# ml-inory/whisper.axera

Hardware: AMD Instinct MI355X
Metric: clips_per_sec (30 s clips, greedy decode, whisper-small) (higher is better)
Workload: dtype bf16; 1 GPU; whisper-small bf16, batch 1/GPU, 30 s synthetic 16 kHz clips resident in HBM, greedy decode 444 ids/clip (448 decoder steps); batch_per_gpu=1, global_batch=1, parallelism=dp1, weights=seeded synthetic, collective=none

## Files before the change

### whisper.axera_amd/csrc/common.hpp

```cpp
#pragma once

#include <hip/hip_runtime.h>
#include <stdint.h>

#ifndef AXW_F16
#define AXW_F16 0
#endif
#if AXW_F16
#define AXW_NS hf
#else
#define AXW_NS bf
#endif

namespace axw {
inline namespace AXW_NS {

#if AXW_F16
typedef _Float16 h16;
constexpr const char* kDtypeName = "fp16";
#else
typedef __bf16 h16;
constexpr const char* kDtypeName = "bf16";
#endif
typedef h16 h16x4 __attribute__((ext_vector_type(4)));
// ... 289 lines not shown
  float* amax_val; int* amax_idx; int amax_stride;
  float* logits_dump; long logits_dump_stride;
  int skip_before_step;
  int ksplit; int part_batch;
};
void launch_decode_gemm(const DecGemmParams& p, hipStream_t s);

struct DecCGemmParams {
  const h16* W;
  const float* bias; int N, K, batch;
  const float* x; const float* ln_w; const float* ln_b;
  const h16* a_hi; const h16* a_lo;
  int nbs;
  int epilogue;
  int rt;
  float* out;
  h16* out_hi; h16* out_lo;
  h16* k_cache; h16* v_cache; long kv_batch_stride; int d_model; int n_ctx_pad;
  const DecState* state;
  const int* off;
  int fold_row0;
  const float* ln_w2;
  const h16* W_lo;
  float* out2;
  float* stat_part;
  unsigned long long* stamp; int stamp_point;
};
void launch_decode_cgemm(const DecCGemmParams& p, hipStream_t s);
int decode_gemm_grid(int N, int rt);
bool decode_logits_resident_ok(int K, int batch);
void launch_act_prep(float* x, const float* g, const float* be, h16* hi, h16* lo, int batch, int K, bool do_ln, int nbs,
                     const float* part, int n_part, int part_batch, const float* part_bias, hipStream_t s);
void launch_pack_weight_frag(const h16* w, h16* wp, int N, int K, hipStream_t s);
void launch_pack_weight_frag_split(const float* w, h16* hi, h16* lo, int N, int K, hipStream_t s);

struct AdvanceParams {
  const float* amax_val; const int* amax_idx; int n_part; int amax_stride;
  DecState* state; int* off; int* tok; int* done; int* n_out; int* out_ids; int batch;
  int* done_host;
  int n_ctx, eot, max_new, n_vocab;
  const int* max_new_clip;
  const int* sot;
  const int* forced; int n_forced;
  int* argmax_dump;
  const h16* tok_emb; const float* pos; float* x; int d_model;
  int n_prefix;
};
void launch_advance(const AdvanceParams& p, hipStream_t s);

struct TsRulesParams {
  const float* logits; long stride;
  int batch, n_vocab, eot, ts_begin;
  const int* off;
  int n_prefix;
  const int* done;
  const int* out_ids; const int* n_out; int n_ctx;
  const int* forced; int n_forced;
  float* amax_val; int* amax_idx; int amax_stride;
};
void launch_timestamp_rules(const TsRulesParams& p, hipStream_t s);

typedef unsigned long long u64;
struct PersistParams {
  const h16* wl; const float* fl;
  const float* qf;
  const h16* tok_emb; const float* pos; const float* ln_w; const float* ln_b;
  const h16* cross_k; const h16* cross_v; long cross_layer_stride;
  int n_layer, n_vocab, n_ctx, n_audio_ctx;
  int eot, max_new, total_steps;
  const int* sot;
  const int* forced; int n_forced; float* logits_dump; int* argmax_dump;
  u64* gran; unsigned* err;
  int gran_bytes;
  int* out_ids; int* n_out; DecState* state;
  int fault;
  long long* prof;
  int n_clip;
  int prof_clip;
  long cross_clip_stride;
  h16* self_k1; h16* self_v1;
  long gran_clip_u64;
  int* out_ids1; int* n_out1; int max_new1;
  int max_new2; long self_clip_stride;
};
bool decode_persistent_supported(int d_model, int n_head, int n_layer, int n_cu);
int decode_persistent_grid(int d_model, int n_cu);
size_t decode_persistent_gran_bytes(int d_model, int grid);
size_t qfold_floats(int d_model, int n_layer);
void launch_qfold_build(const h16* wl, const float* fl, float* qf, int d_model, int n_layer, hipStream_t s);
hipError_t launch_decode_persistent(const PersistParams& p, int d_model, int grid, hipStream_t s);
int decode_persistent_max_clips(int d_model, int n_head, int n_layer, int grid);

void launch_convert_to_h16(const void* src, int src_dtype , h16* dst, long n, hipStream_t s);
void launch_convert_to_f32(const void* src, int src_dtype, float* dst, long n, hipStream_t s);
void launch_conv_weight_pack(const void* src, int src_dtype, h16* dst, int cout, int cin, int kpad, hipStream_t s);

}
}
```

### whisper.axera_amd/csrc/decode_persistent.hip

```cpp
#include "decode_persistent_common.hpp"

namespace axw {
inline namespace AXW_NS {

__global__ void qfold_vec_kernel(const h16* __restrict__ wl, const float* __restrict__ fl, float* __restrict__ qf, int D) {
  const int l = blockIdx.y;
  const long DD = (long)D * D;
  const h16* WL = wl + (long)l * DecArena::w_stride(D);
  const float* F = fl + (long)l * DecArena::f_stride(D);
  float* out = qf + (long)l * qfold_stride(D) + DD;
  const int j = blockIdx.x * blockDim.x + threadIdx.x;
  if (j < 3 * D) {
    const h16* w = WL + DecArena::W_QKV * DD + (long)j * D;
    const float *g = F + DecArena::F_ATTN_LN_W * D, *be = F + DecArena::F_ATTN_LN_B * D;
    double ss = 0.0, cc = 0.0;
    for (int i = 0; i < D; ++i) { const double wv = (double)(float)w[i]; ss += wv * (double)g[i]; cc += wv * (double)be[i]; }
    out[QF_SQKV * D + j] = (float)ss;
    out[QF_CQKV * D + j] = (float)(cc + (double)F[DecArena::F_B_QKV * D + j]);
  }
  if (j < 4 * D) {
    const h16* w = WL + DecArena::W_FC1 * DD + (long)j * D;
    const float *g = F + DecArena::F_MLP_LN_W * D, *be = F + DecArena::F_MLP_LN_B * D;
    double ss = 0.0, cc = 0.0;
    for (int i = 0; i < D; ++i) { const double wv = (double)(float)w[i]; ss += wv * (double)g[i]; cc += wv * (double)be[i]; }
    out[QF_SFC1 * D + j] = (float)ss;
    out[QF_CFC1 * D + j] = (float)(cc + (double)F[DecArena::F_B_FC1 * D + j]);
  }
}


__global__ void qfold_build_kernel(const h16* __restrict__ wl, const float* __restrict__ fl, float* __restrict__ qf, int D) {
  const int l = blockIdx.z;
  const long DD = (long)D * D;
  const h16* wq = wl + (long)l * DecArena::w_stride(D) + DecArena::W_CQ * DD;
  const h16* wo = wl + (long)l * DecArena::w_stride(D) + DecArena::W_O * DD;
  const float* F = fl + (long)l * DecArena::f_stride(D);
  const float *g = F + DecArena::F_CROSS_LN_W * D, *be = F + DecArena::F_CROSS_LN_B * D, *bo = F + DecArena::F_B_O * D, *bq = F + DecArena::F_B_CQ * D;
  float* out = qf + (long)l * qfold_stride(D);
  const int k = blockIdx.x * blockDim.x + threadIdx.x, j = blockIdx.y;
  if (k >= D) return;
  double acc = 0.0;
  for (int i = 0; i < D; ++i) acc += (double)(float)wq[(long)j * D + i] * (double)g[i] * (double)(float)wo[(long)i * D + k];
  out[(long)j * D + k] = (float)acc;
  if (k == 0) {
    double dd = 0.0, ss = 0.0, cc = 0.0;
    for (int i = 0; i < D; ++i) {
      const double w = (double)(float)wq[(long)j * D + i];
      dd += w * (double)g[i] * (double)bo[i];
      ss += w * (double)g[i];
      cc += w * (double)be[i];
    }
    out[DD + j] = (float)dd;
    out[DD + D + j] = (float)ss;
    out[DD + 2 * D + j] = (float)(cc + (double)bq[j]);
  }
}
void launch_qfold_build(const h16* wl, const float* fl, float* qf, int d_model, int n_layer, hipStream_t s) {
  qfold_build_kernel<<<dim3((d_model + 127) / 128, d_model, n_layer), 128, 0, s>>>(wl, fl, qf, d_model);
  qfold_vec_kernel<<<dim3((4 * d_model + 127) / 128, n_layer), 128, 0, s>>>(wl, fl, qf, d_model);
}
size_t qfold_floats(int d_model, int n_layer) { return (size_t)n_layer * (size_t)qfold_stride(d_model); }

template <int LD, int CD, int LF, int CF, bool PROF, bool QF>
__global__ __launch_bounds__(PT) void decode_persistent_kernel(PersistParams p) {
  AXW_PERSIST_SHAPES
  constexpr int XG = D, X0R = 2 * D, A0S = 3 * D;
  AXW_PERSIST_LDS(4)
  AXW_PERSIST_IDS
  const __amdgpu_buffer_rsrc_t GR = __builtin_amdgcn_make_buffer_rsrc((void*)p.gran, 0, p.gran_bytes, 0x27000);
  AXW_PERSIST_ROLES
  AXW_PERSIST_INIT
#define AXW_TL(IDX) \
  if (PROF && tl_on && (tid == 0 || tid == PL)) prof_acc[32 + (IDX)] = wall_clock64();
  int tok = AXW_COLD(sot)[0];
  int n_out = 0, n_done = 0, steps_run = 0;

  if (poller) {
    float x[GD];
    float lg[GD], lb[GD];
    float shift = 0.f;
    AXW_POLLER_PREFETCH
#define AXW_PAIRS_D(BASE) [&](int j) { const int pr = tid + j * PL; return 2 * pr < D ? (BASE) + 2 * pr : -1; }

#define AXW_RAW_STAGE(FAIL, CODE, XGW)                                                      \
  {                                                                                          \
    float s1 = 0.f, s2 = 0.f;                                                                \
    _Pragma("unroll") for (int k = 0; k < GD; ++k) {                                         \
      const int i = el(k);                                                                   \
      if (i < D) {                                                                           \
        const float t = x[k] - shift;                                                        \
        s1 += t; s2 += t * t;                                                                \
        act[i] = x[k] * lg[k];                                                               \
        if (XGW) { act[XG + i] = x[k] * g2[k]; act[X0R + i] = x[k]; }                        \
      }                                                                                      \
    }                                                                                        \
    s1 = wsum(s1); s2 = wsum(s2);                                                            \
    if ((tid & 63) == 0) { red[2 * (tid >> 6)] = s1; red[2 * (tid >> 6) + 1] = s2; }         \
    if (tid == 0) red[2 * NPW + 1] = shift;                                                  \
    if (FAIL) ctl[0] = 1;                                                                    \
    AXW_BARRIER_CHECK(CODE)                                                                  \
    float t1 = 0.f;                                                                          \
    _Pragma("unroll") for (int w2 = 0; w2 < NPW; ++w2) t1 += red[2 * w2];                    \
    shift += t1 / D;                                                                         \
    if (tid == 0) red[2 * NPW] = shift;                                                      \
  }
#define AXW_LN_STAGE(Y, ADD, FAIL, CODE) AXW_LN_STAGE_X(Y, ADD, FAIL, CODE, false)
#define AXW_LN_STAGE_X(Y, ADD, FAIL, CODE, XGW)                                             \
  {                                                                                          \
    float s1 = 0.f, s2 = 0.f;                                                                \
    _Pragma("unroll") for (int k = 0; k < GD; ++k) {                                         \
      if (el(k) < D) {                                                                       \
        if (ADD) x[k] += __uint_as_float(Y[k]);                                              \
        const float t = x[k] - shift;                                                        \
        s1 += t; s2 += t * t;                                                                \
      }                                                                                      \
    }                                                                                        \
    s1 = wsum(s1); s2 = wsum(s2);                                                            \
    if ((tid & 63) == 0) { red[2 * (tid >> 6)] = s1; red[2 * (tid >> 6) + 1] = s2; }         \
    if (FAIL) ctl[0] = 1;                                                                    \
    AXW_BARRIER_CHECK(CODE)                                                                  \
    float t1 = 0.f, t2 = 0.f;                                                                \
    _Pragma("unroll") for (int w2 = 0; w2 < NPW; ++w2) { t1 += red[2 * w2]; t2 += red[2 * w2 + 1]; } \
    const float dm = t1 / D, var = fmaxf(t2 / D - dm * dm, 0.f);                             \
    const float mean = shift + dm, rstd = rsqrtf(var + 1e-5f);                               \
    if (QF && tid == 0) red[2 * NPW] = mean;                                                 \
    _Pragma("unroll") for (int k = 0; k < GD; ++k) {                                         \
      const int i = el(k);                                                                   \
      if (i < D) act[i] = (x[k] - mean) * rstd * lg[k] + lb[k];                              \
      if (QF && (XGW) && i < D) { act[XG + i] = x[k] * g2[k]; act[X0R + i] = x[k]; }         \
    }                                                                                        \
    shift = mean;                                                                            \
    wg_barrier();                                                                            \
  }

    for (int step = 0; step < p.total_steps; ++step) {
      AXW_EMBED(x, tok)
      ln_prefetch(p.fl + DecArena::F_ATTN_LN_W * D, p.fl + DecArena::F_ATTN_LN_B * D);

      for (int l = 0; l < L; ++l) {
        asm volatile("" : "+v"(tid));
        const bool tl_on = step == p.total_steps / 2 && l == L / 2;
        const float* FL = p.fl + (long)l * DecArena::f_stride(D);
        const unsigned tag = (unsigned)(step * L + l + 1);
        {
          unsigned y[GD];
          bool fail = false;
          if (l > 0) fail = gather2<GPD>(GR, tag - 1, y, p.err, ctl, AXW_PAIRS_D(O_Y3));
          AXW_STAMP(0)
          AXW_TL(0)
          if constexpr (QF) {
            if (l > 0) {
#pragma unroll
              for (int k = 0; k < GD; ++k) if (el(k) < D) x[k] += __uint_as_float(y[k]);
            }
            AXW_RAW_STAGE(fail, 0x100 + l, in_o)
            ln_prefetch(FL + DecArena::F_MLP_LN_W * D, FL + DecArena::F_MLP_LN_B * D);
          } else {
            AXW_LN_STAGE_X(y, l > 0, fail, 0x100 + l, in_o)
            ln_prefetch(FL + DecArena::F_CROSS_LN_W * D, FL + DecArena::F_CROSS_LN_B * D);
          }
          AXW_STAMP(1)
          AXW_TL(1)
        }
        if (l == sa_layer) {
// ... 58 lines not shown
              qs[32 + tid] = lo;
            }
            if (fail) ctl[0] = 1;
          }
          AXW_STAMP(7)
          AXW_BARRIER_CHECK(0x500 + l)
          AXW_STAMP(8)
        }
        if (in_o) {
          unsigned y[2 * GP1];
          const bool fail = gather2<GP1>(GR, tag, y, p.err, ctl, [&](int j) { const int pi = tid + j * PL; return pi < NPP1 ? O_PART + (pi / (kPS / 2)) * kRec + 2 * (pi % (kPS / 2)) : -1; });
          float* pbuf = act + D;
#pragma unroll
          for (int j = 0; j < GP1; ++j) {
            const int pi = tid + j * PL;
            if (pi < NPP1) { pbuf[2 * pi] = __uint_as_float(y[2 * j]); pbuf[2 * pi + 1] = __uint_as_float(y[2 * j + 1]); }
          }
          if (fail) ctl[0] = 1;
          AXW_STAMP(9)
          AXW_TL(5)
          AXW_BARRIER_CHECK(0x600 + l)
#pragma unroll
          for (int k = 0; k < GD; ++k) {
            const int i = tid + k * PL;
            if (i < D) {
              act[i] = merge_cross_records(pbuf, i);
            }
          }
          wg_barrier();
          AXW_STAMP(10)
          AXW_TL(6)
        }
        if constexpr (QF) {
          unsigned y[2 * GD];
          const bool fail = gather2<2 * GPD>(GR, tag, y, p.err, ctl, [&](int j) { const int pr = tid + (j % GPD) * PL; return 2 * pr < D ? (j < GPD ? O_Y1 : O_Y2) + 2 * pr : -1; });
#pragma unroll
          for (int k = 0; k < GD; ++k) if (el(k) < D) x[k] = (x[k] + __uint_as_float(y[k])) + __uint_as_float(y[GD + k]);
          AXW_STAMP(11)
          AXW_TL(7)
          AXW_RAW_STAGE(fail, 0x700 + l, false)
          if (l + 1 < L) ln_prefetch(FL + DecArena::f_stride(D) + DecArena::F_ATTN_LN_W * D, FL + DecArena::f_stride(D) + DecArena::F_ATTN_LN_B * D);
          else ln_prefetch(AXW_COLD(ln_w), AXW_COLD(ln_b));
          g2_prefetch(l + 1 < L ? l + 1 : 0);
          AXW_STAMP(12)
          AXW_TL(8)
        } else {
          unsigned y[GD];
          const bool fail = gather2<GPD>(GR, tag, y, p.err, ctl, AXW_PAIRS_D(O_Y2));
          AXW_STAMP(11)
          AXW_TL(7)
          AXW_LN_STAGE(y, true, fail, 0x700 + l)
          if (l + 1 < L) ln_prefetch(FL + DecArena::f_stride(D) + DecArena::F_ATTN_LN_W * D, FL + DecArena::f_stride(D) + DecArena::F_ATTN_LN_B * D);
          else ln_prefetch(AXW_COLD(ln_w), AXW_COLD(ln_b));
          AXW_STAMP(12)
          AXW_TL(8)
        }
        if (in_f2) {
          constexpr int GH = (F / 4 + PL - 1) / PL;
          unsigned y[2 * GH];
          const bool fail = gather2<GH>(GR, tag, y, p.err, ctl, [&](int j) { const int pi = tid + j * PL; return pi < F / 4 ? O_HID + 2 * pi : -1; });
#pragma unroll
          for (int j = 0; j < GH; ++j) {
            const int pi = tid + j * PL;
            if (pi < F / 4) { act[2 * pi] = __uint_as_float(y[2 * j]); act[2 * pi + 1] = __uint_as_float(y[2 * j + 1]); }
          }
          if (fail) ctl[0] = 1;
          AXW_STAMP(13)
          AXW_TL(9)
          AXW_BARRIER_CHECK(0x800 + l)
        }
      }

      steps_run = step + 1;
      asm volatile("" : "+v"(tid));
      if (step < 3) {
        tok = AXW_COLD(sot)[step + 1];
        if constexpr (QF) wg_barrier();
        continue;
      }
      {
        unsigned y[GD];
        const bool fail = gather2<GPD>(GR, (unsigned)(step * L + L), y, p.err, ctl, AXW_PAIRS_D(O_Y3));
        AXW_LN_STAGE(y, true, fail, 0x900)
        AXW_STAMP(14)
        wg_barrier();
        unsigned v[2];
        const bool fail2 = gather2<1>(GR, (unsigned)(step + 1), v, p.err, ctl, [&](int) { return tid < P ? O_AMAX + 2 * tid : -1; });
        float cv = tid < P ? __uint_as_float(v[0]) : -INFINITY;
        int ci = tid < P ? (int)v[1] : 0x7fffffff;
        wave_argmax(cv, ci);
        if ((tid & 63) == 0) { am_v[tid >> 6] = cv; am_i[tid >> 6] = ci; }
        if (fail2) ctl[0] = 1;
        AXW_STAMP(15)
        AXW_BARRIER_CHECK(0xA00)
      }
      float cv = am_v[0];
      int best_idx = am_i[0];
      for (int w2 = 1; w2 < NPW; ++w2)
        if (am_v[w2] > cv || (am_v[w2] == cv && am_i[w2] < best_idx)) { cv = am_v[w2]; best_idx = am_i[w2]; }
      if ((unsigned)best_idx >= (unsigned)AXW_COLD(n_vocab)) best_idx = 0;
      wg_barrier();
      const int gi = step - 3;
      if (AXW_COLD(forced)) {
        if (wg == 0 && tid == 0 && AXW_COLD(argmax_dump) && gi <= AXW_COLD(n_forced)) AXW_COLD(argmax_dump)[gi] = best_idx;
        if (gi < AXW_COLD(n_forced)) tok = AXW_COLD(forced)[gi];
      } else {
        if (best_idx == AXW_COLD(eot) || step + 1 >= AXW_COLD(n_ctx) || n_out >= AXW_COLD(max_new)) { n_done = 1; break; }
        if (wg == 0 && tid == 0) AXW_COLD(out_ids)[n_out] = best_idx;
        ++n_out;
        tok = best_idx;
      }
    }
#undef AXW_LN_STAGE
#undef AXW_LN_STAGE_X
#undef AXW_RAW_STAGE
#undef AXW_PAIRS_D
  } else {
    __builtin_amdgcn_s_setprio(3);
    int ctid = tid - PL;
    constexpr int SLD = CT / LD, NP_Q = (3 * D + SLD - 1) / SLD, NP_F = (F + SLD - 1) / SLD;
    const int pk_qkv = NP_Q <= P ? P - NP_Q : -1;
    const int pk_f = (NP_D + NP_F <= P && NP_Q <= P && NP_D + NP_F + NP_Q >= P) ? NP_D : ((NP_F <= P && NP_Q <= P && NP_F + NP_Q >= P) ? 0 : -1);
    const bool is_fc1 = pk_f < 0 || (rwg >= pk_f && rwg < pk_f + NP_F);
    constexpr bool kEarlyFc2 = CF <= 6;
    const bool early_fc2 = kEarlyFc2 && in_f2 && !is_fc1;
    const int pk_d = 0;
    RowSet<LD, CD> ra, rb;
    RowSet<LF, CF> rs_fc2;
    auto qkv_prefetch = [&](int ly) {
      const h16* w = p.wl + (long)ly * DecArena::w_stride(D);
      if constexpr (QF) {
        const float* v = AXW_COLD(qf) + (long)ly * qfold_stride(D) + (long)D * D;
        ra.prefetch_ln(w, v + QF_SQKV * D, v + QF_CQKV * D, D, 3 * D, rwg, P, ctid, pk_qkv);
      } else {
        ra.prefetch(w, p.fl + (long)ly * DecArena::f_stride(D) + DecArena::F_B_QKV * D, D, 3 * D, rwg, P, ctid, pk_qkv);
      }
    };
    auto stage_stats = [&](float& mean, float& rstd) {
      float t1 = 0.f, t2 = 0.f;
#pragma unroll
      for (int w2 = 0; w2 < NPW; ++w2) { t1 += red[2 * w2]; t2 += red[2 * w2 + 1]; }
      const float dm = t1 / D, var = fmaxf(t2 / D - dm * dm, 0.f);
      mean = red[2 * NPW + 1] + dm;
      rstd = rsqrtf(var + 1e-5f);
    };
    qkv_prefetch(0);
    {
      const int cu0 = ca_unit_of(0, NU, wg, NS);
      if (cu0 >= 0) {
        const int lane = ctid & 63, cw = __builtin_amdgcn_readfirstlane(ctid >> 6);
        const long off = (long)(cu0 / kCrossSplit) * 24 * 4096 + (long)((cu0 % kCrossSplit) * NCW + cw) * 4096;
        for (int i = 0; i < 8; ++i) {
          __builtin_amdgcn_global_load_lds((gptr_t)(p.cross_k + off + i * 512 + lane * 8), (lds_ptr_t)(sK + cw * 4096 + i * 512), 16, 0, kKvAux);
          __builtin_amdgcn_global_load_lds((gptr_t)(p.cross_v + off + i * 512 + lane * 8), (lds_ptr_t)(sV + cw * 4096 + i * 512), 16, 0, kKvAux);
        }
      }
    }

    for (int step = 0; step < p.total_steps; ++step) {
      for (int l = 0; l < L; ++l) {
        asm volatile("" : "+v"(ctid));
        const bool tl_on = step == p.total_steps / 2 && l == L / 2;
        const int lane = ctid & 63, cw = __builtin_amdgcn_readfirstlane(ctid >> 6);
        constexpr long DD = (long)D * D;
        const h16* WL = p.wl + (long)l * DecArena::w_stride(D);
        const float* FL = p.fl + (long)l * DecArena::f_stride(D);
// ... 137 lines not shown
          const float* v = AXW_COLD(qf) + (long)l * qfold_stride(D) + (long)D * D;
          ra.prefetch_ln(w_fc1, v + QF_SFC1 * D, v + QF_CFC1 * D, D, F, rwg, P, ctid, pk_f);
        } else {
          ra.prefetch(w_fc1, b_fc1, D, F, rwg, P, ctid, pk_f);
        }
        if constexpr (kEarlyFc2) {
          if (early_fc2) rs_fc2.prefetch(w_fc2, b_fc2, F, D, rwg, P, ctid, pk_d);
        }
        kv_piece(8, 11);
        AXW_STAMP(25)
        AXW_TL(15)
        AXW_BARRIER_CHECK(0x700 + l)
        if constexpr (QF) {
          AXW_STAMP(26)
          AXW_TL(22)
          float mean, rstd;
          stage_stats(mean, rstd);
          const float* v = AXW_COLD(qf) + (long)l * qfold_stride(D) + (long)D * D;
          ra.run_ln(w_fc1, v + QF_SFC1 * D, v + QF_CFC1 * D, D, act, ctid, res, mean, rstd);
        } else {
          wg_barrier();
          AXW_STAMP(26)
          AXW_TL(22)
          ra.run(w_fc1, b_fc1, D, act, ctid, res);
        }
        ra.publish(ctid, res, pk, ctl + 2, G + O_HID, tag, [](float v) { return gelu_erf(v); });
        if (!early_fc2) rs_fc2.prefetch(w_fc2, b_fc2, F, D, rwg, P, ctid, pk_d);
        kv_piece(11, 13);
        AXW_STAMP(27)
        AXW_TL(16)
        if (in_f2) {
          {
            constexpr int GH = (F / 4 + CT - 1) / CT;
            unsigned y[2 * GH];
            const bool fail = gather2<GH>(GR, tag, y, p.err, ctl, [&](int j) { const int pi = ctid + j * CT; return pi < F / 4 ? O_HID + F / 2 + 2 * pi : -1; });
#pragma unroll
            for (int j = 0; j < GH; ++j) {
              const int pi = ctid + j * CT;
              if (pi < F / 4) { act[F / 2 + 2 * pi] = __uint_as_float(y[2 * j]); act[F / 2 + 2 * pi + 1] = __uint_as_float(y[2 * j + 1]); }
            }
            if (fail) ctl[0] = 1;
          }
          AXW_BARRIER_CHECK(0x800 + l)
          AXW_STAMP(28)
          AXW_TL(23)
          rs_fc2.run(w_fc2, b_fc2, F, act, ctid, res);
          rs_fc2.publish(ctid, res, pk, ctl + 2, G + O_Y3, tag, [](float v) { return v; });
          AXW_STAMP(31)
        }
        if (l + 1 < L) qkv_prefetch(l + 1);
        else if (step >= 3) ra.prefetch(AXW_COLD(tok_emb), nullptr, D, AXW_COLD(n_vocab), rwg, P, ctid);
        else qkv_prefetch(0);
        kv_piece(13, 16);
        AXW_STAMP(29)
        AXW_TL(17)
      }

      steps_run = step + 1;
      asm volatile("" : "+v"(ctid));
      if (step < 3) {
        tok = AXW_COLD(sot)[step + 1];
        if constexpr (QF) wg_barrier();
        continue;
      }
      {
        constexpr int SD = CT / LD;
        const int lane = ctid & 63, cw = __builtin_amdgcn_readfirstlane(ctid >> 6);
        const int N = AXW_COLD(n_vocab);
        const int slot = ctid / LD, j = ctid % LD;
        AXW_BARRIER_CHECK(0x900)
        wg_barrier();
        constexpr bool kActInRegs = CD <= 3;
        float4 a[kActInRegs ? CD : 1][2];
        if constexpr (kActInRegs) {
#pragma unroll
          for (int i = 0; i < CD; ++i) {
            a[i][0] = *reinterpret_cast<const float4*>(act + (j + LD * i) * 8);
            a[i][1] = *reinterpret_cast<const float4*>(act + (j + LD * i) * 8 + 4);
          }
        }
        float bv = -INFINITY;
        int bi = 0x7fffffff;
        float* dump = AXW_COLD(logits_dump) ? AXW_COLD(logits_dump) + (long)(step - 3) * N : nullptr;
        const int r0 = ra.r0, r1 = ra.r1;
        auto consume = [&](const u32x4 (&wr)[CD], int row) {
          float acc;
          if constexpr (kActInRegs) acc = rows_dot_reg<LD, CD>(wr, a);
          else acc = rows_dot<LD, CD>(wr, act, ctid);
          if (j == 0) {
            if (dump) dump[row] = acc;
            if (acc > bv) { bv = acc; bi = row; }
          }
        };
        if constexpr (CD <= 3) {
          u32x4 wn[CD];
          {
            const int nrow = r0 + slot + SD;
            rows_load<LD, CD, kVocabNT>(wn, AXW_COLD(tok_emb), D, nrow < r1 ? nrow : r0, ctid);
          }
          for (int row = r0 + slot; row < r1; row += SD) {
            u32x4 wr[CD];
#pragma unroll
            for (int i = 0; i < CD; ++i) { wr[i] = ra.w[i]; ra.w[i] = wn[i]; }
            const int nrow = row + 2 * SD;
            rows_load<LD, CD, kVocabNT>(wn, AXW_COLD(tok_emb), D, nrow < r1 ? nrow : r0, ctid);
            consume(wr, row);
          }
        } else {
          for (int row = r0 + slot; row < r1; row += SD) {
            u32x4 wr[CD];
#pragma unroll
            for (int i = 0; i < CD; ++i) wr[i] = ra.w[i];
            const int nrow = row + SD;
            rows_load<LD, CD, kVocabNT>(ra.w, AXW_COLD(tok_emb), D, nrow < r1 ? nrow : r0, ctid);
            consume(wr, row);
          }
        }
        qkv_prefetch(0);
        if (j != 0) { bv = -INFINITY; bi = 0x7fffffff; }
        wave_argmax(bv, bi);
        if (lane == 0) { am_v[8 + cw] = bv; am_i[8 + cw] = bi; }
        wg_barrier();
        if (ctid == 0) {
          for (int w2 = 1; w2 < NCW; ++w2)
            if (am_v[8 + w2] > bv || (am_v[8 + w2] == bv && am_i[8 + w2] < bi)) { bv = am_v[8 + w2]; bi = am_i[8 + w2]; }
          am_v[8] = bv; am_i[8] = bi;
        }
        __builtin_amdgcn_wave_barrier();
        if (ctid < 2)
          gput_u(G + O_AMAX + 2 * wg + ctid, (unsigned)(step + 1), ctid == 0 ? __float_as_uint(am_v[8]) : (unsigned)am_i[8]);
        AXW_STAMP(30)
        AXW_BARRIER_CHECK(0xA00)
      }
      float cv = am_v[0];
      int best_idx = am_i[0];
      for (int w2 = 1; w2 < NPW; ++w2)
        if (am_v[w2] > cv || (am_v[w2] == cv && am_i[w2] < best_idx)) { cv = am_v[w2]; best_idx = am_i[w2]; }
      if ((unsigned)best_idx >= (unsigned)AXW_COLD(n_vocab)) best_idx = 0;
      wg_barrier();
      const int gi = step - 3;
      if (AXW_COLD(forced)) {
        if (gi < AXW_COLD(n_forced)) tok = AXW_COLD(forced)[gi];
      } else {
        if (best_idx == AXW_COLD(eot) || step + 1 >= AXW_COLD(n_ctx) || n_out >= AXW_COLD(max_new)) { n_done = 1; break; }
        ++n_out;
        tok = best_idx;
      }
    }
  }

  AXW_PERSIST_DRAIN
  if (wg == 0 && tid == 0) {
    AXW_COLD(n_out)[0] = n_out;
    AXW_COLD(state)->step = steps_run;
    AXW_COLD(state)->n_done = n_done;
  }
#undef AXW_TL
}

int decode_persistent_grid(int d_model, int n_cu) {
  int g = n_cu < d_model ? n_cu : d_model;
  return g < 256 ? g : 256;
}
bool decode_persistent_supported(int d_model, int n_head, int n_layer, int n_cu) {
  if (n_head * 64 != d_model) return false;
  const int P = decode_persistent_grid(d_model, n_cu);
  if (P - n_layer * n_head < 2 * kCrossSplit * n_head) return false;
  return persist_dispatch(d_model, [](auto) { return hipSuccess; }) == hipSuccess;
}
int decode_persistent_max_clips(int d_model, int n_head, int n_layer, int grid) {
  if (d_model > 768) return 1;
  int nc = 1;
  while (nc < 3 && grid - n_layer * n_head >= (nc + 1) * kCrossSplit * n_head && persist_lds_bytes(d_model, nc + 1) <= 160 * 1024) ++nc;
  return nc;
}
size_t decode_persistent_gran_bytes(int d_model, int ) { return ((size_t)16 * d_model + 512 + (size_t)d_model + 64) * 8; }

template <int LD, int CD, int LF, int CF>
static hipError_t launch_one(const PersistParams& p, int grid, hipStream_t s) {
  constexpr int D = 8 * LD * CD;
  if constexpr (D <= 768) {
    if (p.qf)
      return launch_persistent(p.prof ? decode_persistent_kernel<LD, CD, LF, CF, true, true> : decode_persistent_kernel<LD, CD, LF, CF, false, true>, D, 1, p, grid, s);
  }
  return launch_persistent(p.prof ? decode_persistent_kernel<LD, CD, LF, CF, true, false> : decode_persistent_kernel<LD, CD, LF, CF, false, false>, D, 1, p, grid, s);
}

hipError_t launch_decode_persistent(const PersistParams& p, int d_model, int grid, hipStream_t s) {
  if (p.n_clip >= 2) return launch_decode_persistent2(p, d_model, grid, s);
  return persist_dispatch(d_model, [&](auto sh) {
    using S = decltype(sh);
    return launch_one<S::LD, S::CD, S::LF, S::CF>(p, grid, s);
  });
}

}
}
```

### whisper.axera_amd/csrc/engine.cpp

```cpp
#include "engine_impl.hpp"

#include "host_io.hpp"

namespace axw {
inline namespace AXW_NS {

static int dtype_code(const std::string& d) { return d == "F32" ? 0 : d == "BF16" ? 1 : 2; }

static float h16_bits_to_float(uint16_t bits) {
#if AXW_F16
  _Float16 h;
  memcpy(&h, &bits, 2);
  return (float)h;
#else
  const uint32_t u = (uint32_t)bits << 16;
  float f;
  memcpy(&f, &u, 4);
  return f;
#endif
}

Engine::Engine(const std::string& model_type, const std::string& model_path, const std::string& language, int device,
               int max_batch) {
  try {
    construct(model_type, model_path, language, device, max_batch);
  } catch (...) {
    destroy();
    throw;
  }
}

void Engine::construct(const std::string& model_type, const std::string& model_path, const std::string& language, int device,
                       int max_batch) {
  int n_dev = 0;
  if (hipGetDeviceCount(&n_dev) != hipSuccess || n_dev == 0)
    throw std::runtime_error("no HIP device visible: the MI355X engine has no CPU fallback");
  if (device < 0) {
    const char* e = getenv("AX_WHISPER_DEVICE");
    device = e ? atoi(e) : 0;
  }
  if (device >= n_dev) throw std::runtime_error("HIP device ordinal out of range");
  device_ = device;
  const std::string dir = model_path + "/" + model_type;
  load_config(dir, model_type, language);
  tokens_ = load_token_table(dir + "/" + model_type + "-tokens.txt");
  load_t2s(model_path);
  SafeTensors weights_file(dir + "/" + model_type + ".safetensors");
  (void)weights_file.page_in();
  std::lock_guard<std::recursive_mutex> capture_lock(device_capture_mutex(device_));
  HIP_CHECK(hipSetDevice(device_));
  device_set_ = true;
  HIP_CHECK(hipStreamCreateWithFlags(&own_stream_, hipStreamNonBlocking));
  for (auto& e : ev_) HIP_CHECK(hipEventCreate(&e));
  HIP_CHECK(hipStreamCreateWithFlags(&branch_stream_[0], hipStreamNonBlocking));
  HIP_CHECK(hipStreamCreateWithFlags(&admit_stream_, hipStreamNonBlocking));
  HIP_CHECK(hipStreamCreateWithFlags(&copy_stream_, hipStreamNonBlocking));
  if (const char* e = getenv("AX_WHISPER_PAD_STREAMS")) {
    for (int i = 0; i < atoi(e) && i < 8; ++i) {
      hipStream_t pad = nullptr;
      HIP_CHECK(hipStreamCreateWithFlags(&pad, hipStreamNonBlocking));
      pad_streams_.push_back(pad);
    }
  }
  for (auto& e : ev_ring_) HIP_CHECK(hipEventCreateWithFlags(&e, hipEventDisableTiming));
  for (auto& e : ev_step_) HIP_CHECK(hipEventCreateWithFlags(&e, hipEventDisableTiming));
  HIP_CHECK(hipEventCreateWithFlags(&ev_upload_, hipEventDisableTiming));
  HIP_CHECK(hipEventCreateWithFlags(&ev_fork_, hipEventDisableTiming));
  for (auto& e : ev_join_) HIP_CHECK(hipEventCreateWithFlags(&e, hipEventDisableTiming));

  load_weights(weights_file);

  if (max_batch <= 0) {
    const char* e = getenv("AX_WHISPER_MAX_BATCH");
    max_batch = e ? atoi(e) : 1;
  }
  HIP_CHECK(hipHostMalloc((void**)&h_poll_, 64 * sizeof(int), hipHostMallocDefault));
  {
    hipDeviceProp_t prop;
    HIP_CHECK(hipGetDeviceProperties(&prop, device_));
    n_cu_ = prop.multiProcessorCount;
    const char* mode = getenv("AX_WHISPER_DECODE");
    const bool want = !(mode && std::string(mode) == "graph");
    persistent_ok_ = want && decode_persistent_supported(cfg_.n_text_state, cfg_.n_text_head, cfg_.n_text_layer, prop.multiProcessorCount);
    if (persistent_ok_) {
      persist_grid_ = decode_persistent_grid(cfg_.n_text_state, prop.multiProcessorCount);
      gran_bytes_ = decode_persistent_gran_bytes(cfg_.n_text_state, persist_grid_);
      d_gran_ = (u64*)dalloc(3 * gran_bytes_, true);
      allocs_.push_back(d_gran_);
      const char* e2 = getenv("AX_WHISPER_PERSIST2");
      persist_max_clips_ = decode_persistent_max_clips(cfg_.n_text_state, cfg_.n_text_head, cfg_.n_text_layer, persist_grid_);
      if (e2 && e2[0] >= '0' && e2[0] <= '9') persist_max_clips_ = std::max(1, std::min(persist_max_clips_, atoi(e2)));
      {
        const char* eq = getenv("AX_WHISPER_QFOLD");
        if (cfg_.n_text_state <= 768 && !(eq && eq[0] == '0')) {
          d_qfold_ = (float*)dalloc(qfold_floats(cfg_.n_text_state, cfg_.n_text_layer) * sizeof(float));
          allocs_.push_back(d_qfold_);
          launch_qfold_build(dec_w_arena_, dec_f_arena_, d_qfold_, cfg_.n_text_state, cfg_.n_text_layer, own_stream_);
          HIP_CHECK(hipStreamSynchronize(own_stream_));
        }
      }
      if (persist_max_clips_ >= 2) {
        self1_bytes_ = (size_t)cfg_.n_text_layer * cfg_.n_text_head * 8 * 4096 * 2;
        d_self_k1_ = (h16*)dalloc((persist_max_clips_ - 1) * self1_bytes_, true);
        d_self_v1_ = (h16*)dalloc((persist_max_clips_ - 1) * self1_bytes_, true);
        allocs_.push_back(d_self_k1_);
        allocs_.push_back(d_self_v1_);
      }
    }
  }
  cfg_.ints["persistent_two_clips"] = persist_max_clips_ >= 2 ? 1 : 0;
  cfg_.ints["persistent_max_clips"] = persist_max_clips_;
  cfg_.ints["persistent_decode"] = persistent_ok_ ? 1 : 0;
  cfg_.ints["persistent_qfold"] = d_qfold_ ? 1 : 0;
  cfg_.ints["persistent_giveups"] = 0;
  {
    const char* e = getenv("AX_WHISPER_BATCHED_LN");
    const int d = cfg_.n_text_state;
    batched_ln_ = !(e && e[0] == '0') && d % 128 == 0 && (d <= 1024 || (e && e[0] == '2' && d <= 1280));
    cfg_.ints["batched_ln"] = batched_ln_ ? 1 : 0;
    build_cblock_fold();
  }
  {
    enc_split_k_ = true;
    if (const char* t = getenv("AX_WHISPER_GEMV_MAX")) gemv_max_ = std::max(1, std::min(4, atoi(t)));
    if (const char* t = getenv("AX_WHISPER_CROSS_SPLIT")) cross_split_env_ = atoi(t);
    if (const char* t = getenv("AX_WHISPER_ENC_RESCALE_THR")) enc_rescale_thr_ = std::max(0.f, std::min(16.f, (float)atof(t)));
  }
  cfg_.ints["t2s"] = t2s_ ? 1 : 0;
  cfg_.ints["fp16"] = AXW_F16;
  ensure_capacity(std::max(1, max_batch));
  HIP_CHECK(hipStreamSynchronize(own_stream_));
}

Engine::~Engine() { destroy(); }

void Engine::destroy() {
  if (!device_set_) return;
  std::lock_guard<std::recursive_mutex> capture_lock(device_capture_mutex(device_));
  (void)hipSetDevice(device_);
  (void)hipDeviceSynchronize();
  free_slot_buffers();
  for (void* p : allocs_) (void)hipFree(p);
  allocs_.clear();
  if (load_stage_) { (void)hipFree(load_stage_); load_stage_ = nullptr; }
  if (d_over_) { (void)hipFree(d_over_); d_over_ = nullptr; over_cap_ = 0; }
  free_long_arena();
  if (h_poll_) { (void)hipHostFree(h_poll_); h_poll_ = nullptr; }
  for (auto& e : ev_) if (e) { (void)hipEventDestroy(e); e = nullptr; }
  for (auto& e : ev_join_) if (e) { (void)hipEventDestroy(e); e = nullptr; }
  if (ev_fork_) { (void)hipEventDestroy(ev_fork_); ev_fork_ = nullptr; }
  for (auto& b : branch_stream_) if (b) { (void)hipStreamDestroy(b); b = nullptr; }
  if (admit_stream_) { (void)hipStreamDestroy(admit_stream_); admit_stream_ = nullptr; }
  if (copy_stream_) { (void)hipStreamDestroy(copy_stream_); copy_stream_ = nullptr; }
  for (auto& ps : pad_streams_) (void)hipStreamDestroy(ps);
  pad_streams_.clear();
  for (auto& e : ev_ring_) if (e) { (void)hipEventDestroy(e); e = nullptr; }
  for (auto& e : ev_step_) if (e) { (void)hipEventDestroy(e); e = nullptr; }
  if (ev_upload_) { (void)hipEventDestroy(ev_upload_); ev_upload_ = nullptr; }
  if (h_admit_ring_) { (void)hipHostFree(h_admit_ring_); h_admit_ring_ = nullptr; }
  for (auto& e : ev_admit_) if (e) (void)hipEventDestroy(e);
  ev_admit_.clear();
  if (h_done_live_) { (void)hipHostFree(h_done_live_); h_done_live_ = nullptr; }
  if (own_stream_) { (void)hipStreamDestroy(own_stream_); own_stream_ = nullptr; }
}

void* Engine::dalloc(size_t bytes, bool zero) {
  void* p = nullptr;
  HIP_CHECK(hipMalloc(&p, std::max<size_t>(bytes, 256)));
  if (zero) {
    hipError_t e = hipMemset(p, 0, std::max<size_t>(bytes, 256));
    if (e == hipSuccess) e = hipDeviceSynchronize();
    if (e != hipSuccess) {
      (void)hipFree(p);
      throw std::runtime_error(std::string("HIP error: ") + hipGetErrorString(e) + " zero-filling a device buffer");
    }
  }
  return p;
}

void Engine::load_config(const std::string& dir, const std::string& type, const std::string& language) {
  JsonValue j = JsonParser(read_text_file(dir + "/" + type + "_config.json")).parse();
  for (auto& kv : j.obj)
    if (kv.second.kind == JsonValue::Number) cfg_.ints[kv.first] = kv.second.as_int();
  auto geti = [&](const char* k) { return (int)j.at(k).as_int(); };
  {
    std::string fm = j.has("feature_mode") && j.at("feature_mode").kind == JsonValue::String ? j.at("feature_mode").as_str() : "axera_cpp";
    if (const char* e = getenv("AX_WHISPER_FEATURE_MODE")) fm = e;
    if (fm != "axera_cpp" && fm != "openai") throw std::runtime_error("feature_mode must be axera_cpp or openai, not '" + fm + "'");
    feature_openai_ = fm == "openai";
    cfg_.ints["feature_mode_openai"] = feature_openai_ ? 1 : 0;
  }
  cfg_.n_mels = geti("n_mels");
  cfg_.n_vocab = geti("n_vocab");
  cfg_.n_text_state = geti("n_text_state");
  cfg_.n_text_ctx = geti("n_text_ctx");
  cfg_.n_text_layer = geti("n_text_layer");
// ... 763 lines not shown
```

### whisper.axera_amd/csrc/engine.hpp

```cpp
#pragma once

#include <map>
#include <mutex>
#include <string>
#include <vector>

#include "common.hpp"
#include "iengine.hpp"
#include "t2s.hpp"

namespace axw {
class SafeTensors;
inline namespace AXW_NS {

class Engine final : public IEngine {
 public:
  Engine(const std::string& model_type, const std::string& model_path, const std::string& language, int device, int max_batch);
  ~Engine() override;
  Engine(const Engine&) = delete;

  void run_tokens(const float* const* pcm, const float* d_pcm, int d_stride, const int* n_samples, int batch, int max_new,
                  int32_t* ids, int* n_ids, const int* max_new_clip = nullptr) override;
  std::string detokenize(const int32_t* ids, int n) const override;
  std::string transcript(const int32_t* ids, int n) const override;
// ... 99 lines not shown
  hipEvent_t ev_fork_ = nullptr, ev_join_[kMaxBranches - 1] = {nullptr, nullptr, nullptr};
  std::vector<void*> allocs_;
  std::vector<void*> slot_allocs_;

  h16 *conv1_w_ = nullptr, *conv2_w_ = nullptr, *w_cross_kv_ = nullptr, *tok_emb_ = nullptr;
  float *conv1_b_ = nullptr, *conv2_b_ = nullptr, *enc_pos_ = nullptr, *ln_post_w_ = nullptr, *ln_post_b_ = nullptr;
  float *b_cross_kv_ = nullptr, *dec_pos_ = nullptr, *dec_ln_w_ = nullptr, *dec_ln_b_ = nullptr;
  int conv1_k_ = 0;
  std::vector<EncLayer> enc_;
  std::vector<DecLayerW> dec_;
  h16* dec_w_arena_ = nullptr; float* dec_f_arena_ = nullptr;
  struct DecLayerWP { const h16 *w_qkv, *w_o, *w_cq, *w_co, *w_fc1, *w_fc2; h16 *m_hi, *m_lo; };
  struct CblockFold { float *b_qkv4, *b_o2; const float *s, *c; };
  std::vector<CblockFold> cfold_;
  bool cfold_all_ = false;
  float *d_a0_ = nullptr, *d_statp_ = nullptr;
  void build_cblock_fold();
  std::vector<DecLayerWP> dec_packed_;
  const h16* tok_emb_packed_ = nullptr;
  int nbs_ = 1;
  float *twiddle_ = nullptr, *window_ = nullptr, *mel_basis_t_ = nullptr;
  int* d_sot_ = nullptr;

  int cap_ = 0;
  int t_pad_ = 1536, mel_rows_ = 3004, h1_rows_ = 3002;
  float* d_pcm_ = nullptr; long pcm_stride_ = 0; float* h_pcm_ = nullptr;
  float* d_over_ = nullptr; size_t over_cap_ = 0; long long* d_over_off_ = nullptr; bool over_used_ = false;
  int* d_nsamp_ = nullptr; unsigned* d_gmax_ = nullptr; float* d_logmel_ = nullptr; float* d_mel_ref_ = nullptr;
  h16 *d_mel_tm_ = nullptr, *d_h1_ = nullptr, *d_ln_ = nullptr, *d_q_ = nullptr, *d_k_ = nullptr, *d_vt_ = nullptr,
       *d_attn_ = nullptr, *d_ffn_ = nullptr;
  float* d_x_ = nullptr;
  static constexpr int kCrossSplitMax = 6;
  static constexpr int kEncPartClips = 2;
  float* d_enc_part_ = nullptr;
  bool enc_split_k_ = true;
  float enc_rescale_thr_ = 8.f;
  int gemv_max_ = 2;
  int cross_split_env_ = 0;
  h16 *d_cross_k_ = nullptr, *d_cross_v_ = nullptr, *d_self_k_ = nullptr, *d_self_v_ = nullptr;
  float *d_xdec_ = nullptr, *d_qdec_ = nullptr, *d_hid_ = nullptr, *d_part_self_ = nullptr, *d_part_cross_ = nullptr;
  h16 *d_act_[2] = {nullptr, nullptr}, *d_att_[2] = {nullptr, nullptr}, *d_hidp_[2] = {nullptr, nullptr};
  float* d_part_ = nullptr;
  float* d_amax_val_ = nullptr; int* d_amax_idx_ = nullptr; int n_amax_part_ = 0;
  float* d_attn_mpart_ = nullptr;
  unsigned* d_attn_mcnt_ = nullptr;
  int *d_tok_ = nullptr, *d_done_ = nullptr, *d_done_none_ = nullptr, *d_nout_ = nullptr, *d_out_ids_ = nullptr, *d_max_new_clip_ = nullptr;
  int* d_off_ = nullptr;
  int n_cu_ = 0;
  enum SlotState : int { kIdle = 0, kEncoding = 1, kActive = 2, kFinished = 3 };
  int stream_slots_ = 0;
  int stream_user_slots_ = 0;
  std::vector<int> slot_state_, slot_max_new_;
  std::vector<hipEvent_t> ev_admit_;
  hipStream_t admit_stream_ = nullptr;
  int* h_done_live_ = nullptr; int* d_done_live_ = nullptr;
  hipEvent_t ev_step_[3] = {nullptr, nullptr, nullptr};
  long step_seq_ = 0;
  hipStream_t copy_stream_ = nullptr;
  int* d_slot_map_ = nullptr;
  static constexpr int kAdmitRing = 4;
  int* h_admit_ring_ = nullptr;
  hipEvent_t ev_ring_[kAdmitRing] = {nullptr, nullptr, nullptr, nullptr};
  hipEvent_t ev_upload_ = nullptr;
  long admit_seq_ = 0;
  void require_no_stream(const char* what) const;
  DecState* d_state_ = nullptr;
  int* h_poll_ = nullptr;
  int split_self_ = 2, split_cross_ = 6;
  int step_mask_ = 15;
  struct StampMeta { int layer, cross, b0, nb; };
  static constexpr size_t kStampWgs = 4096, kStampLaunches = 256;
  unsigned long long* d_stamp_ = nullptr;
  std::vector<StampMeta> stamp_meta_;
  unsigned long long* next_stamp(int layer, int cross, int b0, int nb);
  bool batched_ln_ = false;
  bool persistent_ok_ = false;
  int persist_max_clips_ = 1;
  h16 *d_self_k1_ = nullptr, *d_self_v1_ = nullptr; size_t self1_bytes_ = 0;
  int persist_skip_ = 0, persist_backoff_ = 0, persist_giveups_ = 0;
  bool persistent_usable();
  void persistent_gave_up();
  void persistent_succeeded();
  int persist_grid_ = 0;
  u64* d_gran_ = nullptr; size_t gran_bytes_ = 0;
  float* d_qfold_ = nullptr;
  std::map<long, hipGraphExec_t> graphs_;
  hipEvent_t ev_[5] = {nullptr, nullptr, nullptr, nullptr, nullptr};
};

}
}
```

### whisper.axera_amd/csrc/engine_decode.cpp

```cpp
#include "engine_impl.hpp"

namespace axw {
inline namespace AXW_NS {

void Engine::reset_decode_state(int batch, const int* max_new_clip) {
  hipStream_t s = stream();
  {
    std::vector<int> mn(batch, cfg_.n_text_ctx);
    if (max_new_clip)
      for (int b = 0; b < batch; ++b) mn[b] = max_new_clip[b] > 0 ? max_new_clip[b] : cfg_.n_text_ctx;
    HIP_CHECK(hipMemcpyAsync(d_max_new_clip_, mn.data(), (size_t)batch * 4, hipMemcpyHostToDevice, s));
    HIP_CHECK(hipStreamSynchronize(s));
  }
  HIP_CHECK(hipMemsetAsync(d_state_, 0, sizeof(DecState), s));
  HIP_CHECK(hipMemsetAsync(d_done_, 0, (size_t)batch * 4, s));
  HIP_CHECK(hipMemsetAsync(d_off_, 0, (size_t)batch * 4, s));
  HIP_CHECK(hipMemsetAsync(d_nout_, 0, (size_t)batch * 4, s));
  std::vector<int> t0(batch, sot_seq_[0]);
  HIP_CHECK(hipMemcpyAsync(d_tok_, t0.data(), (size_t)batch * 4, hipMemcpyHostToDevice, s));
  launch_embed(tok_emb_, dec_pos_, d_tok_, d_off_, d_xdec_, batch, cfg_.n_text_state, s);
  HIP_CHECK(hipStreamSynchronize(s));
}

void Engine::enqueue_decode_step(int batch, int max_new, const int* d_forced, int n_forced, float* d_logits,
// ... 452 lines not shown
  const int n_prefix = ts_mode_ ? 3 : 4;
  if (max_new <= 0 || max_new > Tc - n_prefix) max_new = Tc - n_prefix;
  const bool usable = !ts_mode_ && batch <= std::max(2, persist_max_clips_) && persistent_usable();
  if (usable && batch >= 2 && batch <= persist_max_clips_) {
    int mn[3] = {max_new, -1, -1};
    for (int b = 0; b < batch; ++b) mn[b] = (max_new_clip && max_new_clip[b] > 0) ? std::min(max_new, max_new_clip[b]) : max_new;
    const int st = run_persistent(mn[0], nullptr, 0, nullptr, nullptr, 0, mn[1], mn[2]);
    if (st >= 0) { persistent_succeeded(); return st; }
    persistent_gave_up();
  } else if (usable && batch <= 2) {
    int steps = 0, b = 0;
    for (; b < batch; ++b) {
      int mn = max_new;
      if (max_new_clip && max_new_clip[b] > 0) mn = std::min(mn, max_new_clip[b]);
      const int st = run_persistent(mn, nullptr, 0, nullptr, nullptr, b);
      if (st < 0) break;
      steps = std::max(steps, st);
    }
    if (b == batch) { persistent_succeeded(); return steps; }
    persistent_gave_up();
  }
  hipGraphExec_t g = step_graph(batch, max_new);
  reset_decode_state(batch, max_new_clip);
  hipStream_t s = stream();
  const int total = std::min(Tc, 4 + max_new);
  const int kPoll = 8;
  hipEvent_t pe[2] = {ev_[3], ev_[4]};
  int steps = 0, polls = 0;
  for (int st = 0; st < total; ++st) {
    HIP_CHECK(hipGraphLaunch(g, s));
    ++steps;
    if ((st + 1) % kPoll == 0 && st >= 4) {
      if (polls >= 1) {
        HIP_CHECK(hipEventSynchronize(pe[(polls - 1) & 1]));
        if (h_poll_[(polls - 1) & 1] >= batch) break;
      }
      HIP_CHECK(hipMemcpyAsync(&h_poll_[polls & 1], &d_state_->n_done, 4, hipMemcpyDeviceToHost, s));
      HIP_CHECK(hipEventRecord(pe[polls & 1], s));
      ++polls;
    }
  }
  return steps;
}

int Engine::run_persistent(int max_new, const int* d_forced, int n_forced, float* d_logits, int* d_argmax, int slot, int max_new1, int max_new2) {
  std::lock_guard<std::mutex> launch_lock(persistent_launch_mutex(device_));
  hipStream_t s = stream();
  const int Tc = cfg_.n_text_ctx, H = cfg_.n_text_head;
  PersistParams p{};
  p.wl = dec_w_arena_; p.fl = dec_f_arena_;
  p.qf = d_qfold_;
  p.tok_emb = tok_emb_; p.pos = dec_pos_; p.ln_w = dec_ln_w_; p.ln_b = dec_ln_b_;
  p.cross_k = d_cross_k_ + (size_t)slot * H * t_pad_ * 64;
  p.cross_v = d_cross_v_ + (size_t)slot * H * t_pad_ * 64;
  p.cross_layer_stride = (long)cap_ * H * t_pad_ * 64;
  p.n_layer = cfg_.n_text_layer; p.n_vocab = cfg_.n_vocab; p.n_ctx = Tc; p.n_audio_ctx = cfg_.n_audio_ctx;
  p.eot = cfg_.eot; p.max_new = max_new;
  p.total_steps = d_forced || d_logits || d_argmax ? 4 + n_forced : std::min(Tc, 4 + std::max(max_new, std::max(max_new1, max_new2)));
  p.n_clip = 1;
  if (max_new1 >= 0) {
    p.n_clip = max_new2 >= 0 ? 3 : 2;
    if (persist_max_clips_ < p.n_clip || d_forced || d_logits || d_argmax || slot + p.n_clip > cap_) throw std::runtime_error("run_persistent: that many clips are unsupported here");
    p.cross_clip_stride = (long)H * t_pad_ * 64;
    p.self_k1 = d_self_k1_; p.self_v1 = d_self_v1_;
    p.gran_clip_u64 = (long)(gran_bytes_ / 8);
    p.out_ids1 = d_out_ids_ + (size_t)(slot + 1) * Tc; p.n_out1 = d_nout_ + slot + 1; p.max_new1 = max_new1;
    p.max_new2 = max_new2; p.self_clip_stride = (long)(self1_bytes_ / 2);
  }
  p.sot = d_sot_;
  p.forced = d_forced; p.n_forced = n_forced; p.logits_dump = d_logits; p.argmax_dump = d_argmax;
  p.gran = d_gran_;
  p.gran_bytes = (int)gran_bytes_;
  p.err = reinterpret_cast<unsigned*>(reinterpret_cast<char*>(d_gran_) + gran_bytes_ - 8);
  p.out_ids = d_out_ids_ + (size_t)slot * Tc; p.n_out = d_nout_ + slot; p.state = d_state_;
  long long* d_prof = nullptr;
  const char* prof_path = getenv("AX_WHISPER_PERSIST_PROF");
  if (prof_path) {
    HIP_CHECK(hipMalloc((void**)&d_prof, (size_t)persist_grid_ * 64 * 8));
    HIP_CHECK(hipMemset(d_prof, 0, (size_t)persist_grid_ * 64 * 8));
  }
  p.prof = d_prof;
  { const char* pc = getenv("AX_WHISPER_PERSIST_PROF_CLIP"); p.prof_clip = pc && pc[0] == '1'; }
  p.fault = getenv("AX_WHISPER_PERSIST_FAULT") ? 1 : 0;
  HIP_CHECK(hipMemsetAsync(d_gran_, 0, p.n_clip * gran_bytes_, s));
  HIP_CHECK(hipMemsetAsync(d_state_, 0, sizeof(DecState), s));
  HIP_CHECK(hipMemsetAsync(d_nout_ + slot, 0, 4 * p.n_clip, s));
  if (p.n_clip >= 2) {
    HIP_CHECK(hipMemsetAsync(d_self_k1_, 0, (p.n_clip - 1) * self1_bytes_, s));
    HIP_CHECK(hipMemsetAsync(d_self_v1_, 0, (p.n_clip - 1) * self1_bytes_, s));
  }
  HIP_CHECK(launch_decode_persistent(p, cfg_.n_text_state, persist_grid_, s));
  HIP_CHECK(hipMemcpyAsync(&h_poll_[8], p.err, 4, hipMemcpyDeviceToHost, s));
  HIP_CHECK(hipMemcpyAsync(&h_poll_[9], &d_state_->step, 4, hipMemcpyDeviceToHost, s));
  HIP_CHECK(hipStreamSynchronize(s));
  if (d_prof) {
    std::vector<long long> hp((size_t)persist_grid_ * 64);
    HIP_CHECK(hipMemcpy(hp.data(), d_prof, hp.size() * 8, hipMemcpyDeviceToHost));
    (void)hipFree(d_prof);
    if (FILE* f = fopen(prof_path, "w")) {
      fprintf(f, "# steps %d grid %d; rows = workgroups, columns 0-31 = phase tick sums, 32-63 = absolute ticks of one layer (100 MHz)\n", h_poll_[9], persist_grid_);
      for (int g = 0; g < persist_grid_; ++g) {
        for (int i = 0; i < 64; ++i) fprintf(f, "%lld ", hp[(size_t)g * 64 + i]);
        fprintf(f, "\n");
      }
      fclose(f);
    }
  }
  if (h_poll_[8] != 0) {
    fprintf(stderr, "[ax_whisper] persistent decode gave up (code 0x%x); falling back to the launch-per-phase path\n", (unsigned)h_poll_[8]);
    return -1;
  }
  return h_poll_[9];
}

void Engine::require_timestamp_vocab() const {
  const int T = cfg_.no_timestamps + 1;
  if (cfg_.n_vocab - T != 1501 || T <= cfg_.eot)
    throw std::runtime_error("timestamp mode needs 1501 timestamp ids after <|notimestamps|> (n_vocab " + std::to_string(cfg_.n_vocab) +
                             ", no_timestamps " + std::to_string(cfg_.no_timestamps) + ")");
}

void Engine::ensure_ts_logits() {
  if (d_ts_logits_) return;
  std::lock_guard<std::recursive_mutex> capture_lock(device_capture_mutex(device_));
  ts_stride_ = ((long)cfg_.n_vocab + 3) / 4 * 4;
  d_ts_logits_ = (float*)dalloc((size_t)cap_ * ts_stride_ * 4, true);
  slot_allocs_.push_back(d_ts_logits_);
}

void Engine::enqueue_timestamp_rules(int batch, const int* d_forced, int n_forced, hipStream_t s) {
  TsRulesParams r{};
  r.logits = d_ts_logits_; r.stride = ts_stride_; r.batch = batch;
  r.n_vocab = cfg_.n_vocab; r.eot = cfg_.eot; r.ts_begin = cfg_.no_timestamps + 1;
  r.off = d_off_; r.n_prefix = 3; r.done = d_forced ? nullptr : d_done_;
  r.out_ids = d_out_ids_; r.n_out = d_nout_; r.n_ctx = cfg_.n_text_ctx;
  r.forced = d_forced; r.n_forced = n_forced;
  r.amax_val = d_amax_val_; r.amax_idx = d_amax_idx_; r.amax_stride = n_amax_part_;
  launch_timestamp_rules(r, s);
}

void Engine::fetch_ids(int batch, int32_t* ids, int* n_ids) {
  hipStream_t s = stream();
  HIP_CHECK(hipMemcpyAsync(ids, d_out_ids_, (size_t)batch * cfg_.n_text_ctx * 4, hipMemcpyDeviceToHost, s));
  HIP_CHECK(hipMemcpyAsync(n_ids, d_nout_, (size_t)batch * 4, hipMemcpyDeviceToHost, s));
  HIP_CHECK(hipStreamSynchronize(s));
}

}
}
```

Baseline: 9.111 clips/s.

## Keep a tail slice of vocab embedding rows resident in poller-wave registers

The poller waves of each workgroup preload the last slice of that workgroup's vocabulary rows of the tied token embedding into VGPRs once at kernel start. At each step they compute those rows' logits and a partial argmax during the final-LN stage, and the streaming logits loop shrinks its row range by that amount. The partial argmax is merged through LDS scratch. This cuts per-step HBM/L2 traffic for the vocabulary projection and overlaps part of it with the LN stage, at the cost of heavy register pressure in the poller path, which may reduce occupancy or cause spills.

```diff
diff --git a/whisper.axera_amd/csrc/common.hpp b/whisper.axera_amd/csrc/common.hpp
--- a/whisper.axera_amd/csrc/common.hpp
+++ b/whisper.axera_amd/csrc/common.hpp
@@ -395,6 +395,7 @@
   long gran_clip_u64;
   int* out_ids1; int* n_out1; int max_new1;
   int max_new2; long self_clip_stride;
+  int vocab_resident;
 };
 bool decode_persistent_supported(int d_model, int n_head, int n_layer, int n_cu);
 int decode_persistent_grid(int d_model, int n_cu);
@@ -403,6 +404,7 @@
 void launch_qfold_build(const h16* wl, const float* fl, float* qf, int d_model, int n_layer, hipStream_t s);
 hipError_t launch_decode_persistent(const PersistParams& p, int d_model, int grid, hipStream_t s);
 int decode_persistent_max_clips(int d_model, int n_head, int n_layer, int grid);
+int decode_persistent_vocab_resident_rows(int d_model, int n_vocab, int grid);
 
 void launch_convert_to_h16(const void* src, int src_dtype , h16* dst, long n, hipStream_t s);
 void launch_convert_to_f32(const void* src, int src_dtype, float* dst, long n, hipStream_t s);
diff --git a/whisper.axera_amd/csrc/decode_persistent.hip b/whisper.axera_amd/csrc/decode_persistent.hip
--- a/whisper.axera_amd/csrc/decode_persistent.hip
+++ b/whisper.axera_amd/csrc/decode_persistent.hip
@@ -61,9 +61,12 @@
 }
 size_t qfold_floats(int d_model, int n_layer) { return (size_t)n_layer * (size_t)qfold_stride(d_model); }
 
+template <int CD, bool PROF>
+constexpr int kVocabRes = CD > 3 ? 0 : PROF ? 5 : 6;
 template <int LD, int CD, int LF, int CF, bool PROF, bool QF>
 __global__ __launch_bounds__(PT) void decode_persistent_kernel(PersistParams p) {
   AXW_PERSIST_SHAPES
+  constexpr int NRES = kVocabRes<CD, PROF>, VCAP = NRES * (PL / LD);
   constexpr int XG = D, X0R = 2 * D, A0S = 3 * D;
   AXW_PERSIST_LDS(4)
   AXW_PERSIST_IDS
@@ -80,6 +83,27 @@
     float lg[GD], lb[GD];
     float shift = 0.f;
     AXW_POLLER_PREFETCH
+    unsigned vres[NRES > 0 ? NRES : 1][4 * CD];
+    auto vocab_tail = [&](int& v0, int& vb, int& v1) {
+      const unsigned N = (unsigned)AXW_COLD(n_vocab);
+      v0 = (int)((unsigned)rwg * N / (unsigned)P);
+      v1 = (int)((unsigned)(rwg + 1) * N / (unsigned)P);
+      vb = AXW_COLD(vocab_resident) ? (v1 - v0 > VCAP ? v1 - VCAP : v0) : v1;
+    };
+    if constexpr (NRES > 0) {
+      int v0, vb, v1;
+      vocab_tail(v0, vb, v1);
+      if (vb == v1) vb = v0;
+#pragma unroll
+      for (int k = 0; k < NRES; ++k) {
+        const int row = vb + k * (PL / LD) + tid / LD;
+        u32x4 w[CD];
+        rows_load<LD, CD>(w, AXW_COLD(tok_emb), D, row < v1 ? row : v0, tid);
+#pragma unroll
+        for (int i = 0; i < 4 * CD; ++i) { vres[k][i] = w[i / 4][i % 4]; asm volatile("" : "+v"(vres[k][i])); }
+      }
+      __builtin_amdgcn_s_waitcnt(0x0F70);
+    }
 #define AXW_PAIRS_D(BASE) [&](int j) { const int pr = tid + j * PL; return 2 * pr < D ? (BASE) + 2 * pr : -1; }
 
 #define AXW_RAW_STAGE(FAIL, CODE, XGW)                                                      \
@@ -304,6 +328,35 @@
         unsigned y[GD];
         const bool fail = gather2<GPD>(GR, (unsigned)(step * L + L), y, p.err, ctl, AXW_PAIRS_D(O_Y3));
         AXW_LN_STAGE(y, true, fail, 0x900)
+        if constexpr (NRES > 0) {
+          int v0, vb, v1;
+          vocab_tail(v0, vb, v1);
+          if (vb < v1) {
+            float* dump = AXW_COLD(logits_dump) ? AXW_COLD(logits_dump) + (long)(step - 3) * AXW_COLD(n_vocab) : nullptr;
+            float bv = -INFINITY;
+            int bi = 0x7fffffff;
+#pragma unroll
+            for (int k = 0; k < NRES; ++k) {
+              u32x4 w[CD];
+#pragma unroll
+              for (int i = 0; i < 4 * CD; ++i) {
+                unsigned t;
+                asm volatile("v_mov_b32 %0, %1" : "=v"(t) : "v"(vres[k][i]));
+                w[i / 4][i % 4] = t;
+              }
+              int tid2 = tid;
+              asm volatile("" : "+v"(tid2));
+              const float acc = rows_dot<LD, CD>(w, act, tid2);
+              const int row = vb + k * (PL / LD) + tid / LD;
+              if (tid % LD == 0 && row < v1) {
+                if (dump) dump[row] = acc;
+                if (acc > bv) { bv = acc; bi = row; }
+              }
+            }
+            wave_argmax(bv, bi);
+            if ((tid & 63) == 0) { pscr[tid >> 6] = bv; reinterpret_cast<int*>(pscr)[NPW + (tid >> 6)] = bi; }
+          }
+        }
         AXW_STAMP(14)
         wg_barrier();
         unsigned v[2];
@@ -607,7 +660,8 @@
         float bv = -INFINITY;
         int bi = 0x7fffffff;
         float* dump = AXW_COLD(logits_dump) ? AXW_COLD(logits_dump) + (long)(step - 3) * N : nullptr;
-        const int r0 = ra.r0, r1 = ra.r1;
+        const int nres = NRES > 0 && AXW_COLD(vocab_resident) ? (ra.r1 - ra.r0 > VCAP ? VCAP : ra.r1 - ra.r0) : 0;
+        const int r0 = ra.r0, r1 = ra.r1 - nres;
         auto consume = [&](const u32x4 (&wr)[CD], int row) {
           float acc;
           if constexpr (kActInRegs) acc = rows_dot_reg<LD, CD>(wr, a);
@@ -649,6 +703,13 @@
         if (ctid == 0) {
           for (int w2 = 1; w2 < NCW; ++w2)
             if (am_v[8 + w2] > bv || (am_v[8 + w2] == bv && am_i[8 + w2] < bi)) { bv = am_v[8 + w2]; bi = am_i[8 + w2]; }
+          if (nres > 0) {
+            for (int w2 = 0; w2 < NPW; ++w2) {
+              const float pv = pscr[w2];
+              const int pi = reinterpret_cast<const int*>(pscr)[NPW + w2];
+              if (pv > bv || (pv == bv && pi < bi)) { bv = pv; bi = pi; }
+            }
+          }
           am_v[8] = bv; am_i[8] = bi;
         }
         __builtin_amdgcn_wave_barrier();
@@ -699,6 +760,16 @@
   while (nc < 3 && grid - n_layer * n_head >= (nc + 1) * kCrossSplit * n_head && persist_lds_bytes(d_model, nc + 1) <= 160 * 1024) ++nc;
   return nc;
 }
+int decode_persistent_vocab_resident_rows(int d_model, int n_vocab, int grid) {
+  int cap = 0;
+  (void)persist_dispatch(d_model, [&](auto sh) {
+    using S = decltype(sh);
+    cap = kVocabRes<S::CD, false> * (PL / S::LD);
+    return hipSuccess;
+  });
+  const int rows = grid > 0 ? n_vocab / grid : 0;
+  return cap < rows ? cap : rows;
+}
 size_t decode_persistent_gran_bytes(int d_model, int ) { return ((size_t)16 * d_model + 512 + (size_t)d_model + 64) * 8; }
 
 template <int LD, int CD, int LF, int CF>
diff --git a/whisper.axera_amd/csrc/engine.cpp b/whisper.axera_amd/csrc/engine.cpp
--- a/whisper.axera_amd/csrc/engine.cpp
+++ b/whisper.axera_amd/csrc/engine.cpp
@@ -99,6 +99,10 @@
           HIP_CHECK(hipStreamSynchronize(own_stream_));
         }
       }
+      {
+        const char* ev = getenv("AX_WHISPER_VOCAB_RESIDENT");
+        if (!(ev && ev[0] == '0')) vocab_resident_rows_ = decode_persistent_vocab_resident_rows(cfg_.n_text_state, cfg_.n_vocab, persist_grid_);
+      }
       if (persist_max_clips_ >= 2) {
         self1_bytes_ = (size_t)cfg_.n_text_layer * cfg_.n_text_head * 8 * 4096 * 2;
         d_self_k1_ = (h16*)dalloc((persist_max_clips_ - 1) * self1_bytes_, true);
@@ -112,6 +116,7 @@
   cfg_.ints["persistent_max_clips"] = persist_max_clips_;
   cfg_.ints["persistent_decode"] = persistent_ok_ ? 1 : 0;
   cfg_.ints["persistent_qfold"] = d_qfold_ ? 1 : 0;
+  cfg_.ints["vocab_resident_rows"] = vocab_resident_rows_;
   cfg_.ints["persistent_giveups"] = 0;
   {
     const char* e = getenv("AX_WHISPER_BATCHED_LN");
diff --git a/whisper.axera_amd/csrc/engine.hpp b/whisper.axera_amd/csrc/engine.hpp
--- a/whisper.axera_amd/csrc/engine.hpp
+++ b/whisper.axera_amd/csrc/engine.hpp
@@ -205,6 +205,7 @@
   void persistent_gave_up();
   void persistent_succeeded();
   int persist_grid_ = 0;
+  int vocab_resident_rows_ = 0;
   u64* d_gran_ = nullptr; size_t gran_bytes_ = 0;
   float* d_qfold_ = nullptr;
   std::map<long, hipGraphExec_t> graphs_;
diff --git a/whisper.axera_amd/csrc/engine_decode.cpp b/whisper.axera_amd/csrc/engine_decode.cpp
--- a/whisper.axera_amd/csrc/engine_decode.cpp
+++ b/whisper.axera_amd/csrc/engine_decode.cpp
@@ -558,6 +558,7 @@
   p.prof = d_prof;
   { const char* pc = getenv("AX_WHISPER_PERSIST_PROF_CLIP"); p.prof_clip = pc && pc[0] == '1'; }
   p.fault = getenv("AX_WHISPER_PERSIST_FAULT") ? 1 : 0;
+  p.vocab_resident = vocab_resident_rows_ > 0 ? 1 : 0;
   HIP_CHECK(hipMemsetAsync(d_gran_, 0, p.n_clip * gran_bytes_, s));
   HIP_CHECK(hipMemsetAsync(d_state_, 0, sizeof(DecState), s));
   HIP_CHECK(hipMemsetAsync(d_nout_ + slot, 0, 4 * p.n_clip, s));
```

Result: faster. 9.291 clips/s, median of 6 (+2.0%).
